# emolch/kiwi

Hardware: AMD Instinct MI355X
Metric: trial-source misfit evals/s (higher is better)
Workload: dtype f32

## Files before the change

### kiwi_amd/csrc/kiwi_accum.hip

```cpp
#include "kiwi_accum_api.hpp"

#if KIWI_ARITH == 0
#define KIWI_ARITH_NS exact
#elif KIWI_ARITH == 1
#define KIWI_ARITH_NS fused
#else
#error "KIWI_ARITH: 0 (exact) or 1 (fused)"
#endif

namespace kiwi {
namespace KIWI_ARITH_NS {

#include "kiwi_accum.inc"

#define KIWI_COMMON_ARGS a.G, a.span, a.pitch, a.recs, a.cent_ofs, a.isrc0, a.nrec, a.recv, a.syn, a.syn_stride

#if KIWI_FAMILY == 1
void launch_direct(const AccumArgs &a, dim3 grid)
{
    if (a.ng == 10) hipLaunchKernelGGL(accumulate_kernel<10>, grid, dim3(256), 0, a.stream, KIWI_COMMON_ARGS, a.synrow);
    else            hipLaunchKernelGGL(accumulate_kernel<8>, grid, dim3(256), 0, a.stream, KIWI_COMMON_ARGS, a.synrow);
}
#endif

// ... 31 lines not shown
template <int NG, int NS, bool COMPACT, bool PLAN>
static void multi_t(const AccumArgs &a, dim3 grid, int ntiles, const int *mate, const int *wider)
{
    if (a.fuse) hipLaunchKernelGGL((accumulate_multi_kernel<NG, true, NS, COMPACT, PLAN>), grid, dim3(256), 0, a.stream, KIWI_COMMON_ARGS, ntiles, a.tab, a.coefs, a.fp,
                                   a.pairflag, mate, wider, a.plan, a.plan_ofs);
    else        hipLaunchKernelGGL((accumulate_multi_kernel<NG, false, NS, COMPACT, PLAN>), grid, dim3(256), 0, a.stream, KIWI_COMMON_ARGS, ntiles, a.tab, a.coefs, a.fp,
                                   a.pairflag, mate, wider, a.plan, a.plan_ofs);
}
template <int NG, int NS>
static void multi_c(const AccumArgs &a, dim3 grid, int ntiles, const int *mate, const int *wider)
{
    if (a.compact && a.plan) multi_t<NG, NS, true, true>(a, grid, ntiles, mate, wider);
    else if (a.compact) multi_t<NG, NS, true, false>(a, grid, ntiles, mate, wider);
    else multi_t<NG, NS, false, false>(a, grid, ntiles, mate, wider);
}
void launch_multi(const AccumArgs &a, dim3 grid, int NS, int ntiles, const int *mate, const int *wider)
{
    if (a.ng == 10) { if (NS == 4) multi_c<10, 4>(a, grid, ntiles, mate, wider); else multi_c<10, 2>(a, grid, ntiles, mate, wider); }
    else            { if (NS == 4) multi_c<8, 4>(a, grid, ntiles, mate, wider); else multi_c<8, 2>(a, grid, ntiles, mate, wider); }
}
void launch_multi_plan(const AccumArgs &a, int NS, int ngroups, const int *mate, const int *wider, PlanSrc *plan)
{
    const dim3 grid((unsigned)ngroups, (unsigned)((a.nrec + 63) / 64));
    if (NS == 4) hipLaunchKernelGGL(multi_plan_kernel<4>, grid, dim3(64), 0, a.stream, a.recs, a.cent_ofs, a.isrc0, a.nrec, a.recv, a.tab, a.pairflag, mate, wider,
                                    a.plan_ofs, (int4 *)plan, a.plan_regular, a.plan_repeat, a.plan_count);
    else         hipLaunchKernelGGL(multi_plan_kernel<2>, grid, dim3(64), 0, a.stream, a.recs, a.cent_ofs, a.isrc0, a.nrec, a.recv, a.tab, a.pairflag, mate, wider,
                                    a.plan_ofs, (int4 *)plan, a.plan_regular, a.plan_repeat, a.plan_count);
}
#endif

#if KIWI_FAMILY == 4
template <int NG, bool COMPACT>
static void cell_t(const AccumArgs &a, dim3 grid, int ntiles, bool per_wave)
{
#define KIWI_C(KERNEL) hipLaunchKernelGGL(KERNEL, grid, dim3(256), 0, a.stream, KIWI_COMMON_ARGS, ntiles, a.tab, a.coefs, a.fp, a.pairflag, a.synrow, \
                                          a.fam_ofs, a.fam_list)
    if (per_wave) { if (a.fuse) KIWI_C((accumulate_cellw_kernel<NG, true, COMPACT>)); else KIWI_C((accumulate_cellw_kernel<NG, false, COMPACT>)); }
    else          { if (a.fuse) KIWI_C((accumulate_cell_kernel<NG, 256, 2, 0, true, COMPACT>)); else KIWI_C((accumulate_cell_kernel<NG, 256, 2, 0, false, COMPACT>)); }
#undef KIWI_C
}
template <int NG>
static void cell_c(const AccumArgs &a, dim3 grid, int ntiles, bool per_wave)
{
    if (a.compact) cell_t<NG, true>(a, grid, ntiles, per_wave); else cell_t<NG, false>(a, grid, ntiles, per_wave);
}
void launch_cell(const AccumArgs &a, dim3 grid, int ntiles) { if (a.ng == 10) cell_c<10>(a, grid, ntiles, false); else cell_c<8>(a, grid, ntiles, false); }
void launch_cellw(const AccumArgs &a, dim3 grid, int ntiles) { if (a.ng == 10) cell_c<10>(a, grid, ntiles, true); else cell_c<8>(a, grid, ntiles, true); }
int cellw_range() { return kCellwRange; }
#endif
// ... 4 lines not shown
```

### kiwi_amd/csrc/kiwi_accum.inc

```


typedef float f4u __attribute__((ext_vector_type(4), aligned(4)));
typedef float f2u __attribute__((ext_vector_type(2), aligned(4)));

#if defined(KIWI_EXPLICIT_FMA)
#ifndef KIWI_CELLW_AHEAD
#define KIWI_CELLW_AHEAD 3
#endif
template <class V> __device__ __forceinline__ V kiwi_mad(V acc, float w, V v)
{
    V ws;
    for (int k = 0; k < (int)(sizeof(V) / sizeof(float)); k++) ws[k] = w;
    return __builtin_elementwise_fma(ws, v, acc);
}
template <class V> __device__ __forceinline__ V kiwi_madv(V acc, V w, V v) { return __builtin_elementwise_fma(w, v, acc); }
#else
template <class V> __device__ __forceinline__ V kiwi_mad(V acc, float w, V v) { return acc + w * v; }
template <class V> __device__ __forceinline__ V kiwi_madv(V acc, V w, V v) { return acc + w * v; }
#endif

typedef int v4i_t __attribute__((ext_vector_type(4)));
typedef int v2i_t __attribute__((ext_vector_type(2)));
__device__ __forceinline__ __amdgpu_buffer_rsrc_t gf_rsrc(const float *base)
{
// ... 256 lines not shown

template <bool BLEND>
__device__ __forceinline__ void pair_finish(const f4u (&v)[2][BLEND ? 4 : 1], float *__restrict__ tile0, int lds_tile, int ig0, int p,
                                            const GeoRec &g)
{
#pragma unroll
    for (int q = 0; q < 2; q++) {
        f4u b;
        if constexpr (BLEND) {
            b = g.w[0] * v[q][0];
            b = b + g.w[1] * v[q][1];
            b = b + g.w[2] * v[q][2];
            b = b + g.w[3] * v[q][3];
        } else {
            b = v[q][0];
        }
        *(float4 *)(tile0 + (ig0 + q) * lds_tile + p) = make_float4(b.x, b.y, b.z, b.w);
    }
}

struct HaloRegs { f4u v[4]; };

struct DescLanes {
    int ta, tb;
    __device__ __forceinline__ int a(int ig, int k) const { return REC_I(ta, 4 * ig + k); }
    __device__ __forceinline__ int b(int ig, int k) const { return REC_I(tb, 4 * ig + k); }
    __device__ __forceinline__ int ha(int hig, int k) const { return __shfl(ta, 4 * hig + k, 64); }
    __device__ __forceinline__ int hb(int hig, int k) const { return __shfl(tb, 4 * hig + k, 64); }
    __device__ __forceinline__ bool fast(int jb, int lds_tile, int pitch, int lane, int ng) const
    {
        const bool lane_ok = lane >= 4 * ng || (ta + jb >= tb && ta + jb + lds_tile <= tb + pitch);
        return __builtin_amdgcn_ballot_w64(lane_ok) == ~0ull;
    }
};
struct DescPlan {
    int b0[4], o[4], pitch, hoff;
    __device__ __forceinline__ int b(int ig, int k) const { return b0[k] + ig * pitch; }
    __device__ __forceinline__ int a(int ig, int k) const { return b0[k] + ig * pitch + o[k]; }
    __device__ __forceinline__ int hb(int, int k) const { return b0[k] + hoff; }
    __device__ __forceinline__ int ha(int, int k) const { return b0[k] + hoff + o[k]; }
    __device__ __forceinline__ bool fast(int jb, int lds_tile, int pitch_, int, int) const
    {
        const int omin = min(min(o[0], o[1]), min(o[2], o[3])), omax = max(max(o[0], o[1]), max(o[2], o[3]));
        return omin + jb >= 0 && omax + jb + lds_tile <= pitch_;
    }
};

template <bool BLEND, bool FAST, typename D>
__device__ __forceinline__ HaloRegs halo_issue(bool active, int ig, int ph, int jb, const float *__restrict__ G, int pitch, const D &d)
{
    HaloRegs h;
#pragma unroll
    for (int k = 0; k < (BLEND ? 4 : 1); k++) {
        const int base = d.ha(ig, k);
        int idx = base + jb + ph;
        if constexpr (!FAST) {
            const int lo = d.hb(ig, k);
            idx = min(max(idx, lo), lo + pitch - 4);
        }
        h.v[k] = f4u{ 0.f, 0.f, 0.f, 0.f };
        if (active) h.v[k] = *(const f4u *)(G + (size_t)(unsigned)idx);
    }
    return h;
}
template <bool BLEND, bool FAST>
__device__ __forceinline__ HaloRegs halo_issue(bool active, int ig, int ph, int jb, const float *__restrict__ G, int pitch,
// ... 836 lines not shown
        const int base = d.a(ig, k);
        if constexpr (FAST) {
            v[k] = buf_load4(gf_rsrc(G), p, base + jb);
        } else {
            const int lo = d.b(ig, k);
            const int idx = min(max(base + j, lo), lo + pitch - 4);
            v[k] = *(const f4u *)(G + (size_t)(unsigned)idx);
        }
    }
}

template <typename D>
__device__ __forceinline__ void one_issue_hidden(f4u (&v)[4], int ig, int p, int jb, const float *__restrict__ G, const D &d)
{
    const size_t gi = (size_t)G;
    const v4i_t rs = { (int)(unsigned)gi, (int)((unsigned)(gi >> 32) & 0xffffu), -1, 0x00020000 };
    const int voff = (int)(4u * (unsigned)p);
#pragma unroll
    for (int k = 0; k < 4; k++) {
        const int soff = (int)(4u * (unsigned)(d.a(ig, k) + jb));
        asm volatile("buffer_load_dwordx4 %0, %1, %2, %3 offen" : "=v"(v[k]) : "v"(voff), "s"(rs), "s"(soff));
    }
}
template <int CNT_FULL, int CNT_SHORT>
__device__ __forceinline__ void vm_wait(f4u (&v)[4], int full )
{
    if constexpr (CNT_FULL == CNT_SHORT)
        asm volatile("s_waitcnt vmcnt(%4)" : "+v"(v[0]), "+v"(v[1]), "+v"(v[2]), "+v"(v[3]) : "n"(CNT_FULL));
    else
        asm volatile("s_cmp_eq_u32 %6, 0\n\ts_cbranch_scc1 1f\n\ts_waitcnt vmcnt(%4)\n\ts_branch 2f\n1:\n\ts_waitcnt vmcnt(%5)\n2:"
                     : "+v"(v[0]), "+v"(v[1]), "+v"(v[2]), "+v"(v[3]) : "n"(CNT_FULL), "n"(CNT_SHORT), "s"(full) : "scc");
}

template <bool BLEND>
__device__ __forceinline__ void one_finish(const f4u (&v)[BLEND ? 4 : 1], float *__restrict__ tile0, int lds_tile, int ig, int p,
                                           const GeoRec &g)
{
    f4u b;
    if constexpr (BLEND) {
        b = g.w[0] * v[0];
        b = b + g.w[1] * v[1];
        b = b + g.w[2] * v[2];
        b = b + g.w[3] * v[3];
    } else {
        b = v[0];
    }
// ... 28 lines not shown
                 "+v"(v.r[2][0]), "+v"(v.r[2][1]), "+v"(v.r[2][2]), "+v"(v.r[2][3]), "+v"(v.r[3][0]), "+v"(v.r[3][1]), "+v"(v.r[3][2]), "+v"(v.r[3][3])
    if constexpr (CNT_FULL == CNT_SHORT)
        asm volatile("s_waitcnt vmcnt(%16)" : KIWI_R16 : "n"(CNT_FULL));
    else
        asm volatile("s_cmp_eq_u32 %18, 0\n\ts_cbranch_scc1 1f\n\ts_waitcnt vmcnt(%16)\n\ts_branch 2f\n1:\n\ts_waitcnt vmcnt(%17)\n2:"
                     : KIWI_R16 : "n"(CNT_FULL), "n"(CNT_SHORT), "s"(full) : "scc");
#undef KIWI_R16
}
__device__ __forceinline__ void mfma_finish(const RowsDw &v, float *__restrict__ dst, const float (&w)[4], bool write)
{
    const f4m negz = { -0.f, -0.f, -0.f, -0.f };
#pragma unroll
    for (int m = 0; m < 4; m++) {
        f4m b = __builtin_amdgcn_mfma_f32_4x4x1f32(v.r[0][m], w[0], negz, 0, 0, 0);
        b = b + __builtin_amdgcn_mfma_f32_4x4x1f32(v.r[1][m], w[1], negz, 0, 0, 0);
        b = b + __builtin_amdgcn_mfma_f32_4x4x1f32(v.r[2][m], w[2], negz, 0, 0, 0);
        b = b + __builtin_amdgcn_mfma_f32_4x4x1f32(v.r[3][m], w[3], negz, 0, 0, 0);
        if (write) *(float4 *)(dst + 64 * m) = make_float4(b.x, b.y, b.z, b.w);
    }
}

template <int NG, int NS> __host__ __device__ constexpr int multi_set_stride() { return NG * (1024 / NS + kHalo) + ((NS == 4 && KIWI_MFMA_BLEND) ? 8 : 0); }

template <int NG, bool FAST, int NS, typename D, typename Shadow>
__device__ __forceinline__ void multi_build(float *__restrict__ tile0, int wv, int lane, int tid, int jb, const float *__restrict__ G,
                                            int pitch, const D &d, const GeoRec (&gw)[NS], int only, bool hact, bool whalo, int hig, int hph,
                                            Shadow shadow)
{
    constexpr int TILE = 1024 / NS, LDS_TILE = TILE + kHalo, DEPTH = 3, SET = multi_set_stride<NG, NS>();
    constexpr int N = (NS == 2) ? NG / 2 : (NG + 3) / 4;
    const int p = (NS == 2) ? 4 * (64 * (wv & 1) + lane) : 4 * lane;
    auto comp = [&](int i) { return (NS == 2) ? 2 * i + (wv >> 1) : wv + 4 * i; };
    HaloRegs hv;
    if (whalo) hv = halo_issue<true, FAST>(true, hig, hph, jb, G, pitch, d);
    const bool last_ok = comp(N - 1) < NG;
    if constexpr (KIWI_MFMA_BLEND && FAST && NS == 4 && KIWI_ARITH == 0) {
        RowsDw v[N];
#pragma unroll
        for (int i = 0; i < DEPTH && i < N; i++) if (i < N - 1 || last_ok) rows_issue_dw(v[i], comp(i), lane, jb, G, d);
        __syncthreads();
        shadow();
        const int me = lane & 3;
        float w[4];
#pragma unroll
        for (int k = 0; k < 4; k++) w[k] = me == 0 ? gw[0].w[k] : (me == 1 ? gw[1].w[k] : (me == 2 ? gw[2].w[k] : gw[3].w[k]));
        float *__restrict__ dst = tile0 + me * SET + 4 * (lane >> 2);
        const bool write = only < 0 || only == me;
#pragma unroll
        for (int i = 0; i < N; i++) {
            __builtin_amdgcn_sched_barrier(0);
            if (i < N - 1 || last_ok) {
                const int behind = (i + DEPTH < N ? i + DEPTH : N) - 1 - i;
                const bool short_ = behind > 0 && i + DEPTH >= N;
                const int lastf = __builtin_amdgcn_readfirstlane(last_ok ? 1 : 0);
                switch (behind) {
                case 0: vm_wait16<0, 0>(v[i], 1); break;
                case 1: if (short_) vm_wait16<16, 0>(v[i], lastf); else vm_wait16<16, 16>(v[i], 1); break;
                default: if (short_) vm_wait16<32, 16>(v[i], lastf); else vm_wait16<32, 32>(v[i], 1); break;
                }
                mfma_finish(v[i], dst + comp(i) * LDS_TILE, w, write);
            }
            if (i + DEPTH < N && (i + DEPTH < N - 1 || last_ok)) rows_issue_dw(v[i + DEPTH], comp(i + DEPTH), lane, jb, G, d);
        }
        if (whalo) {
#pragma unroll
            for (int s = 0; s < NS; s++)
                if (only < 0 || only == s) halo_finish<true>(hact, hv, tile0 + s * SET, LDS_TILE, hig, hph, gw[s]);
        }
        return;
    }
    f4u v[N][4];
    auto issue = [&](int i) __attribute__((always_inline)) {
        if constexpr (FAST) one_issue_hidden(v[i], comp(i), p, jb, G, d);
        else one_issue<true, false>(v[i], comp(i), p, jb, G, pitch, d);
    };
#pragma unroll
    for (int i = 0; i < DEPTH && i < N; i++) if (i < N - 1 || last_ok) issue(i);
    __syncthreads();
    shadow();
#pragma unroll
    for (int i = 0; i < N; i++) {
        __builtin_amdgcn_sched_barrier(0);
        if (i < N - 1 || last_ok) {
            if constexpr (FAST) {
                const int behind = (i + DEPTH < N ? i + DEPTH : N) - 1 - i;
                const bool short_ = behind > 0 && i + DEPTH >= N;
                const int lastf = __builtin_amdgcn_readfirstlane(last_ok ? 1 : 0);
                switch (behind) {
                case 0: vm_wait<0, 0>(v[i], 1); break;
                case 1: if (short_) vm_wait<4, 0>(v[i], lastf); else vm_wait<4, 4>(v[i], 1); break;
                default: if (short_) vm_wait<8, 4>(v[i], lastf); else vm_wait<8, 8>(v[i], 1); break;
                }
            }
#pragma unroll
            for (int s = 0; s < NS; s++)
                if (only < 0 || only == s) one_finish<true>(v[i], tile0 + s * SET, LDS_TILE, comp(i), p, gw[s]);
        }
        if (i + DEPTH < N && (i + DEPTH < N - 1 || last_ok)) issue(i + DEPTH);
    }
    if (whalo) {
#pragma unroll
        for (int s = 0; s < NS; s++)
            if (only < 0 || only == s) halo_finish<true>(hact, hv, tile0 + s * SET, LDS_TILE, hig, hph, gw[s]);
    }
}


__device__ __forceinline__ int smax_u(int a, int b) { int r; asm("s_max_i32 %0, %1, %2" : "=s"(r) : "s"(a), "s"(b) : "scc"); return r; }
__device__ __forceinline__ int smin_u(int a, int b) { int r; asm("s_min_i32 %0, %1, %2" : "=s"(r) : "s"(a), "s"(b) : "scc"); return r; }

template <int NS>
__device__ __forceinline__ bool multi_taken(const RecvDev &rv, const int *__restrict__ pairflag, const int *__restrict__ mate,
                                            int s, int nrec, int r)
{
    if (!mate) return false;
    const int a = s - s % NS;
    if (!mate[a / NS] || !rv.need_h || !rv.has_d) return false;
    int f = 0;
#pragma unroll
    for (int i = 0; i < NS; i++) f |= pairflag[(size_t)(a + i) * nrec + r];
    return f == 0;
}

template <int NS>
__global__ __launch_bounds__(64) void multi_plan_kernel(const GeoRec *__restrict__ recs, const int *__restrict__ cent_ofs, int isrc0, int nrec,
    const RecvDev *__restrict__ recv, const int *__restrict__ off4, const int *__restrict__ pairflag, const int *__restrict__ mate,
    const int *__restrict__ mate_wider, const int *__restrict__ plan_ofs, int4 *__restrict__ plan,
    int regular_on , int repeat_on ,
    unsigned *__restrict__ count )
{
    constexpr int TILE = 1024 / NS, LDS_TILE = TILE + kHalo;
    const int k = (int)blockIdx.x, s0 = NS * k, r = (int)(blockIdx.y * 64 + threadIdx.x);
    if (r >= nrec) return;
    const RecvDev &rv = recv[r];
    if (!rv.enabled) return;
    if (!multi_taken<NS>(rv, pairflag, mate, s0, nrec, r)) return;
    if constexpr (NS == 2) { if (multi_taken<4>(rv, pairflag, mate_wider, s0, nrec, r)) return; }
    const int cb = cent_ofs[isrc0];
    const int nc = cent_ofs[isrc0 + s0 + 1] - cent_ofs[isrc0 + s0];
    const size_t pbeg = (size_t)plan_ofs[k], pend = (size_t)plan_ofs[k + 1];
    size_t pi = pbeg + (size_t)r;
    for (int c = 0; c < nc && pi < pend; pi += (size_t)nrec) {
        const GeoRec *h[NS];
        int smaxs[NS], smins[NS], npos = 0;
        bool shared = true, same_rows = true;
#pragma unroll
        for (int i = 0; i < NS; i++) {
            h[i] = recs + ((size_t)(cent_ofs[isrc0 + s0 + i] - cb) * nrec + (size_t)r * nc + c);
// ... 18 lines not shown
            }
        }
        const int glen = h[0]->pad & 0xff;
        int4 *__restrict__ out = plan + pi * (kPlanStride / 16);
        unsigned nreg = 0, nrep = 0;
#pragma unroll
        for (int i = 0; i < NS; i++) {
            const int4 o = *(const int4 *)(off4 + ((size_t)(cent_ofs[isrc0 + s0 + i] - cb) * nrec + (size_t)r * nc + c) * 4);
            const int e0 = smaxs[i] - h[i]->ishift;
            bool regular = regular_on != 0 && e0 >= 0 && e0 <= kPlanE0Mask;
            bool steps01 = regular && repeat_on != 0 && glen <= 5;
            int repeats = 0;
            for (int j = 1; j < glen && c + j < nc; j++) {
                const int d = h[i][j].ishift - h[i][j - 1].ishift;
                regular = regular && d == 1;
                steps01 = steps01 && (d == 0 || d == 1);
                if (d == 0 && j <= 4) repeats |= 1 << (j - 1);
            }
            if (regular || !steps01) repeats = 0;
            nreg += regular ? 1u : 0u;
            nrep += repeats ? 1u : 0u;
            const int head = (h[i]->flags & 0xffff) | (regular || repeats ? (e0 << kPlanE0Shift) | (regular ? kPlanRegularBit : 0) | (repeats << kPlanRepeatShift) : 0)
                             | (glen << 16) | ((shared ? 1 : 0) << 23) | ((npos - TILE) << 24);
            out[4 * i + 0] = make_int4(h[i]->row[0], h[i]->row[1], h[i]->row[2], h[i]->row[3]);
            out[4 * i + 1] = o;
            out[4 * i + 2] = make_int4(__float_as_int(h[i]->w[0]), __float_as_int(h[i]->w[1]), __float_as_int(h[i]->w[2]), __float_as_int(h[i]->w[3]));
            out[4 * i + 3] = make_int4(smaxs[i], head, __float_as_int(h[i]->cl), __float_as_int(h[i]->sl));
        }
        if (count) { atomicAdd(count, (unsigned)NS); atomicAdd(count + 1, nreg); atomicAdd(count + 2, nrep); }
        if (glen < 1) break;
        c += glen;
    }
}

typedef const __attribute__((address_space(4))) v4i_t *plan_cptr;
template <int NS>
__device__ __forceinline__ int plan_warm(size_t p)
{
    int d;
    if constexpr (NS == 4)
        asm volatile("s_load_dword %0, %1, 0x0\n\ts_load_dword %0, %1, 0x40\n\ts_load_dword %0, %1, 0x80\n\ts_load_dword %0, %1, 0xc0" : "=&s"(d) : "s"(p) : "memory");
    else
        asm volatile("s_load_dword %0, %1, 0x0\n\ts_load_dword %0, %1, 0x40" : "=&s"(d) : "s"(p) : "memory");
    return d;
}

template <int NG, bool FUSE, int NS, bool COMPACT ,
// ... 45 lines not shown
        const long long b = (long long)(cent_ofs[isrc0 + s0 + i] - cb) * nrec + (long long)r * nc;
        rbase[i] = ((long long)__builtin_amdgcn_readfirstlane((int)(b >> 32)) << 32) | (unsigned)__builtin_amdgcn_readfirstlane((int)b);
    }
    auto recs_of = [&](int i) { return recs + (size_t)rbase[i]; };
    auto tab_of = [&](int i) { return tab + (size_t)rbase[i] * (compact ? 4 : 128); };
    int c = 0;
    int cur[NS];
    int ta = 0, tb = 0;
    if constexpr (!PLAN) {
#pragma unroll
        for (int i = 0; i < NS; i++) cur[i] = rec_load(recs_of(i), 0, nc, lane);
        if constexpr (compact) ta = off4_load(tab_of(0), 0, lane);
        else { ta = tab_of(0)[lane]; tb = tab_of(0)[64 + lane]; }
    }
    const int hq = 255 - tid, hch = min(hq / NG, 15), hig = hq % NG, hph = TILE + 4 * hch;
    size_t pcur = 0;
    if constexpr (PLAN) {
        const size_t a = (size_t)plan + ((size_t)plan_ofs[blockIdx.x] + (size_t)r) * kPlanStride;
        pcur = ((size_t)(unsigned)__builtin_amdgcn_readfirstlane((int)(a >> 32)) << 32) | (unsigned)__builtin_amdgcn_readfirstlane((int)a);
    }
    const int pstep = nrec * kPlanStride;
    const int hoff = PLAN ? hig * pitch : 0;
    auto plan4 = [&](int byte) { return *(plan_cptr)(pcur + (size_t)(unsigned)byte); };
    while (c < nc) {
        GeoRec g[NS];
        int smaxs[NS], smins[NS], npos = 0;
        bool shared = true, same_rows = true;
        int glen_p = 0;
        DescPlan dp;
        if constexpr (PLAN) {
            const v4i_t rw = plan4(0), of = plan4(16), tl = plan4(48);
            g[0].row[0] = rw.x;
            dp = DescPlan{ { 0, (rw.y - rw.x) * pitch, (rw.z - rw.x) * pitch, (rw.w - rw.x) * pitch }, { of.x, of.y, of.z, of.w }, pitch, hoff };
            const unsigned head = (unsigned)tl.y;
            glen_p = (int)((head >> 16) & 0x7fu);
            shared = ((head >> 23) & 1u) != 0u;
            npos = TILE + (int)(head >> 24);
            smaxs[0] = tl.x;
        }
        if constexpr (compact && !PLAN) desc_expand(ta, cur[0], lane, pitch, ta, tb);
        if constexpr (!PLAN) {
#pragma unroll
        for (int i = 0; i < NS; i++) {
            g[i].ishift = REC_I(cur[i], 8);
            g[i].pad = REC_I(cur[i], 19);
            smaxs[i] = g[i].ishift + ((g[i].pad >> 8) & 0xff);
            smins[i] = g[i].ishift - ((g[i].pad >> 16) & 0xff);
            npos = max(npos, TILE + (smaxs[i] - smins[i]) + 8);
            if (i == 0) g[0].row[0] = REC_I(cur[0], 0);
            else {
                same_rows = same_rows && (__builtin_amdgcn_ballot_w64(cur[i] != cur[0]) & 0xfull) == 0ull;
                shared = shared && smaxs[i] == smaxs[0];
            }
        }
        shared = shared && same_rows;
        if (same_rows && !shared) {
            int smax_c = smaxs[0], smin_c = smins[0];
#pragma unroll
            for (int i = 1; i < NS; i++) { smax_c = smax_u(smax_c, smaxs[i]); smin_c = smin_u(smin_c, smins[i]); }
            if (TILE + (smax_c - smin_c) + 8 <= LDS_TILE) {
                shared = true;
                npos = TILE + (smax_c - smin_c) + 8;
#pragma unroll
                for (int i = 0; i < NS; i++) smaxs[i] = smax_c;
            }
        }
        }
        const int glen = PLAN ? glen_p : (g[0].pad & 0xff);
        const int cend = c + glen;
        int smax = smaxs[0];
        if constexpr (PLAN) smax = plan4(64 * sh + 48).x;
        else {
#pragma unroll
            for (int i = 1; i < NS; i++) if (sh == i) smax = smaxs[i];
        }
        int flags = 0, ishv = 0, warm_ = 0, pwarm_ = 0;
        float gcl = 0.f, gsl = 0.f;
        const float *__restrict__ coef_grp = nullptr;
        auto shadow = [&]() {
            if constexpr (PLAN) {
#pragma unroll
                for (int i = 0; i < NS; i++) {
                    const v4i_t w = plan4(64 * i + 32);
                    g[i].w[0] = __int_as_float(w.x); g[i].w[1] = __int_as_float(w.y); g[i].w[2] = __int_as_float(w.z); g[i].w[3] = __int_as_float(w.w);
                }
                const v4i_t me = plan4(64 * sh + 48);
                flags = me.y & 0xffff; gcl = __int_as_float(me.z); gsl = __int_as_float(me.w);
                if (c + glen < nc) pwarm_ = plan_warm<NS>(pcur + (size_t)(unsigned)pstep);
            } else {
#pragma unroll
            for (int i = 0; i < NS; i++) { g[i].w[0] = REC_F(cur[i], 4); g[i].w[1] = REC_F(cur[i], 5); g[i].w[2] = REC_F(cur[i], 6); g[i].w[3] = REC_F(cur[i], 7); }
            int curme = cur[0];
#pragma unroll
            for (int i = 1; i < NS; i++) if (sh == i) curme = cur[i];
            flags = REC_I(curme, 18);
            gcl = REC_F(curme, 16); gsl = REC_F(curme, 17);
            }
            if (!(PLAN && (flags & (kPlanRegularBit | kPlanRepeatMask)))) { if (lane < glen) ishv = rc[c + lane].ishift; }
            const size_t crow = (base_me + c) * kCoefLine;
            const unsigned clo = __builtin_amdgcn_readfirstlane((unsigned)crow), chi = __builtin_amdgcn_readfirstlane((unsigned)(crow >> 32));
            coef_grp = coefs + (((size_t)chi << 32) | clo);
            if constexpr (NG == 10) warm_ = coef_warm(coef_grp);
        };
        auto noshadow = []() {};
#define KIWI_MULTI_BUILD(DESC, I0, ONLY, NPOS, SHADOW) do { \
            const int jb_ = t_tile0 - smaxs[I0] - 1;       \
            const float *__restrict__ Gg = G + (size_t)g[I0].row[0] * (size_t)pitch; \
            const bool fast = (DESC).fast(jb_, LDS_TILE, pitch, lane, NG); \
            const bool hact = hq < 16 * NG && hph < (NPOS); \
            const bool whalo = __builtin_amdgcn_ballot_w64(hact) != 0ull; \
            if (fast) multi_build<NG, true, NS>(&tiles[0], wv, lane, tid, jb_, Gg, pitch, DESC, g, ONLY, hact, whalo, hig, hph, SHADOW); \
            else      multi_build<NG, false, NS>(&tiles[0], wv, lane, tid, jb_, Gg, pitch, DESC, g, ONLY, hact, whalo, hig, hph, SHADOW); } while (0)
        __builtin_amdgcn_s_setprio(1);
        if constexpr (PLAN) {
            if (shared) KIWI_MULTI_BUILD(dp, 0, -1, npos, shadow);
            else {
                KIWI_MULTI_BUILD(dp, 0, 0, npos, shadow);
#pragma unroll
                for (int i = 1; i < NS; i++) {
                    const v4i_t rw = plan4(64 * i), of = plan4(64 * i + 16);
                    smaxs[i] = plan4(64 * i + 48).x;
                    g[i].row[0] = rw.x;
                    const DescPlan di{ { 0, (rw.y - rw.x) * pitch, (rw.z - rw.x) * pitch, (rw.w - rw.x) * pitch }, { of.x, of.y, of.z, of.w }, pitch, hoff };
                    KIWI_MULTI_BUILD(di, i, i, npos, noshadow);
                }
            }
            asm volatile("" :: "s"(pwarm_));
            pcur += (size_t)(unsigned)pstep;
        } else {
        if (shared) KIWI_MULTI_BUILD((DescLanes{ ta, tb }), 0, -1, npos, shadow);
        else {
            KIWI_MULTI_BUILD((DescLanes{ ta, tb }), 0, 0, npos, shadow);
#pragma unroll
            for (int i = 1; i < NS; i++) {
                int tai, tbi;
                if constexpr (compact) desc_expand(off4_load(tab_of(i), c, lane), cur[i], lane, pitch, tai, tbi);
                else { tai = tab_of(i)[(size_t)c * 128 + lane]; tbi = tab_of(i)[(size_t)c * 128 + 64 + lane]; }
                g[i].row[0] = REC_I(cur[i], 0);
                KIWI_MULTI_BUILD((DescLanes{ tai, tbi }), i, i, npos, noshadow);
            }
        }
#pragma unroll
        for (int i = 0; i < NS; i++) cur[i] = rec_load(recs_of(i), cend, nc, lane);
        if (cend < nc) {
            if constexpr (compact) ta = off4_load(tab_of(0), cend, lane);
            else { ta = tab_of(0)[(size_t)cend * 128 + lane]; tb = tab_of(0)[(size_t)cend * 128 + 64 + lane]; }
        }
        }
#undef KIWI_MULTI_BUILD
        __syncthreads();
        __builtin_amdgcn_s_setprio(0);
        {
            const unsigned abase = (unsigned)(size_t)(lds_cfp)&tiles[sh * SET + u0];
            if constexpr (NG == 10 || NG == 8) {
                asm volatile("" :: "s"(warm_));
                const float gcl_u = __int_as_float(__builtin_amdgcn_readfirstlane(__float_as_int(gcl))), gsl_u = __int_as_float(__builtin_amdgcn_readfirstlane(__float_as_int(gsl)));
                const size_t cg_ = (size_t)coef_grp;
                const float *__restrict__ coef_u = (const float *)(((size_t)(unsigned)__builtin_amdgcn_readfirstlane((int)(cg_ >> 32)) << 32) | (unsigned)__builtin_amdgcn_readfirstlane((int)cg_));
                const int n = cend - c;
#define KIWI_ASM_ARGS ar1[0], ar1[1], ar2[0], ar2[1], dz[0], dz[1], abase, ishv, smax, n, coef_u, gcl_u, gsl_u
#define KIWI_PLAN_ARGS ar1[0], ar1[1], ar2[0], ar2[1], dz[0], dz[1], abase, ishv, smax, n, coef_u, gcl_u, gsl_u, head_u
                if constexpr (PLAN) {
                    const int head_u = __builtin_amdgcn_readfirstlane(flags);
                    if constexpr (NG == 10) {
                        if (flags & 2) { if constexpr (K == 5) KIWI_APPLY_PLAN(10, 5, rot)(KIWI_PLAN_ARGS); else KIWI_APPLY_PLAN(10, 9, rot)(KIWI_PLAN_ARGS); }
                        else           { if constexpr (K == 5) KIWI_APPLY_PLAN(10, 5, plain)(KIWI_PLAN_ARGS); else KIWI_APPLY_PLAN(10, 9, plain)(KIWI_PLAN_ARGS); }
                    } else {
                        if (flags & 2) { if constexpr (K == 5) KIWI_APPLY_PLAN(8, 5, rot)(KIWI_PLAN_ARGS); else KIWI_APPLY_PLAN(8, 9, rot)(KIWI_PLAN_ARGS); }
                        else           { if constexpr (K == 5) KIWI_APPLY_PLAN(8, 5, plain)(KIWI_PLAN_ARGS); else KIWI_APPLY_PLAN(8, 9, plain)(KIWI_PLAN_ARGS); }
                    }
                } else
                if constexpr (NG == 10) {
                    if (flags & 2) { if constexpr (K == 5) KIWI_APPLY_ASM(10, 5, rot)(KIWI_ASM_ARGS); else KIWI_APPLY_ASM(10, 9, rot)(KIWI_ASM_ARGS); }
                    else           { if constexpr (K == 5) KIWI_APPLY_ASM(10, 5, plain)(KIWI_ASM_ARGS); else KIWI_APPLY_ASM(10, 9, plain)(KIWI_ASM_ARGS); }
                } else {
                    if (flags & 2) { if constexpr (K == 5) KIWI_APPLY_ASM(8, 5, rot)(KIWI_ASM_ARGS); else KIWI_APPLY_ASM(8, 9, rot)(KIWI_ASM_ARGS); }
                    else           { if constexpr (K == 5) KIWI_APPLY_ASM(8, 5, plain)(KIWI_ASM_ARGS); else KIWI_APPLY_ASM(8, 9, plain)(KIWI_ASM_ARGS); }
                }
#undef KIWI_ASM_ARGS
#undef KIWI_PLAN_ARGS
            } else {
            int cc = c, eprev = 0;
            bool have = false;
#define KIWI_C2STEP(LL, HH, RV, CC) do { \
                const int e = smax - __builtin_amdgcn_readlane(ishv, (CC) - c);        \
                const int d = have ? eprev - e : 0x7fff; \
                carry2_apply<NG, RV, K>(ar1, ar2, dz, LL, HH, abase + 4u * (unsigned)e, d, d, coef_grp + (size_t)((CC) - c) * kCoefLine, gcl, gsl); \
                have = true; eprev = e; } while (0)
            if (flags & 2) {
                set2_dead(X); set2_dead(Y);
                for (; cc + 1 < cend; cc += 2) { KIWI_C2STEP(X, Y, true, cc); KIWI_C2STEP(Y, X, true, cc + 1); }
                if (cc < cend) KIWI_C2STEP(X, Y, true, cc);
            } else {
                set2_dead(X); set2_dead(Y);
                for (; cc + 1 < cend; cc += 2) { KIWI_C2STEP(X, Y, false, cc); KIWI_C2STEP(Y, X, false, cc + 1); }
                if (cc < cend) KIWI_C2STEP(X, Y, false, cc);
            }
#undef KIWI_C2STEP
            }
        }
        c = cend;
    }
    {
        const int js = s0 + sh;
        const int tl = tile * TILE + u0;
        if (!FUSE && tl >= rv.wlen) return;
        float *__restrict__ so = syn + (size_t)js * syn_stride + tl;
        float mom = 0.f;
        if constexpr (FUSE) mom = fp.moment[fp.isrc0 + js];
        const bool whole = tile * TILE + TILE <= rv.wlen;
        for (int k = 0; k < rv.ncomp; k++) {
            f2v o01, o23;
            out4(rv.comp[k], rv.sign[k], rv.cl0, rv.sl0, ar1, ar2, dz, o01, o23);
            if constexpr (!FUSE) {
                const float o[4] = { o01.x, o01.y, o23.x, o23.y };
#pragma unroll
                for (int i = 0; i < 4; i++)
                    if (tl + 64 * i < rv.wlen) so[rv.synofs[k] + 64 * i] = o[i];
                continue;
            }
            double acc = fused_acc4(fp, o01, o23, mom, fp.reft + rv.refofs[k] + tl, fp.tw + rv.refofs[k] + tl, tl, rv.wlen, whole);
            acc = wave_reduce_f64(acc, fp.method == 6);
            if (lane == 63)
// ... 575 lines not shown
```

Baseline: 39180.

## Trim scalar work in planned multi-build: precomputed row offsets, linear loads, coef pointer

The plan kernel now stores row deltas already multiplied by the pitch, so the accumulate kernel no longer recomputes them. A linear-descriptor buffer-load path uses scalar offsets precomputed once per group. The per-group coefficient pointer is advanced incrementally instead of being recomputed with readfirstlane, and the last-task flag and halo threshold are hoisted out of the loop. For the plan path, halo weights are reloaded late and the lane activity test is done lazily, and coef warm is disabled by default. Together these aim to cut scalar ALU work and SGPR pressure in the hot loop, at the cost of more template complexity and a changed plan format.

```diff
diff --git a/kiwi_amd/csrc/kiwi_accum.hip b/kiwi_amd/csrc/kiwi_accum.hip
--- a/kiwi_amd/csrc/kiwi_accum.hip
+++ b/kiwi_amd/csrc/kiwi_accum.hip
@@ -77,9 +77,9 @@
 void launch_multi_plan(const AccumArgs &a, int NS, int ngroups, const int *mate, const int *wider, PlanSrc *plan)
 {
     const dim3 grid((unsigned)ngroups, (unsigned)((a.nrec + 63) / 64));
-    if (NS == 4) hipLaunchKernelGGL(multi_plan_kernel<4>, grid, dim3(64), 0, a.stream, a.recs, a.cent_ofs, a.isrc0, a.nrec, a.recv, a.tab, a.pairflag, mate, wider,
+    if (NS == 4) hipLaunchKernelGGL(multi_plan_kernel<4>, grid, dim3(64), 0, a.stream, a.recs, a.cent_ofs, a.isrc0, a.nrec, a.pitch, a.recv, a.tab, a.pairflag, mate, wider,
                                     a.plan_ofs, (int4 *)plan, a.plan_regular, a.plan_repeat, a.plan_count);
-    else         hipLaunchKernelGGL(multi_plan_kernel<2>, grid, dim3(64), 0, a.stream, a.recs, a.cent_ofs, a.isrc0, a.nrec, a.recv, a.tab, a.pairflag, mate, wider,
+    else         hipLaunchKernelGGL(multi_plan_kernel<2>, grid, dim3(64), 0, a.stream, a.recs, a.cent_ofs, a.isrc0, a.nrec, a.pitch, a.recv, a.tab, a.pairflag, mate, wider,
                                     a.plan_ofs, (int4 *)plan, a.plan_regular, a.plan_repeat, a.plan_count);
 }
 #endif
diff --git a/kiwi_amd/csrc/kiwi_accum.inc b/kiwi_amd/csrc/kiwi_accum.inc
--- a/kiwi_amd/csrc/kiwi_accum.inc
+++ b/kiwi_amd/csrc/kiwi_accum.inc
@@ -302,6 +302,7 @@
 struct HaloRegs { f4u v[4]; };
 
 struct DescLanes {
+    static constexpr bool linear = false;
     int ta, tb;
     __device__ __forceinline__ int a(int ig, int k) const { return REC_I(ta, 4 * ig + k); }
     __device__ __forceinline__ int b(int ig, int k) const { return REC_I(tb, 4 * ig + k); }
@@ -313,7 +314,10 @@
         return __builtin_amdgcn_ballot_w64(lane_ok) == ~0ull;
     }
 };
+__device__ __forceinline__ int smax_u(int a, int b) { int r; asm("s_max_i32 %0, %1, %2" : "=s"(r) : "s"(a), "s"(b) : "scc"); return r; }
+__device__ __forceinline__ int smin_u(int a, int b) { int r; asm("s_min_i32 %0, %1, %2" : "=s"(r) : "s"(a), "s"(b) : "scc"); return r; }
 struct DescPlan {
+    static constexpr bool linear = true;
     int b0[4], o[4], pitch, hoff;
     __device__ __forceinline__ int b(int ig, int k) const { return b0[k] + ig * pitch; }
     __device__ __forceinline__ int a(int ig, int k) const { return b0[k] + ig * pitch + o[k]; }
@@ -321,7 +325,7 @@
     __device__ __forceinline__ int ha(int, int k) const { return b0[k] + hoff + o[k]; }
     __device__ __forceinline__ bool fast(int jb, int lds_tile, int pitch_, int, int) const
     {
-        const int omin = min(min(o[0], o[1]), min(o[2], o[3])), omax = max(max(o[0], o[1]), max(o[2], o[3]));
+        const int omin = smin_u(smin_u(o[0], o[1]), smin_u(o[2], o[3])), omax = smax_u(smax_u(o[0], o[1]), smax_u(o[2], o[3]));
         return omin + jb >= 0 && omax + jb + lds_tile <= pitch_;
     }
 };
@@ -1204,6 +1208,17 @@
         asm volatile("buffer_load_dwordx4 %0, %1, %2, %3 offen" : "=v"(v[k]) : "v"(voff), "s"(rs), "s"(soff));
     }
 }
+__device__ __forceinline__ void one_issue_hidden_linear(f4u (&v)[4], int igp , int p, const float *__restrict__ G, const int (&t)[4])
+{
+    const size_t gi = (size_t)G;
+    const v4i_t rs = { (int)(unsigned)gi, (int)((unsigned)(gi >> 32) & 0xffffu), -1, 0x00020000 };
+    const int voff = (int)(4u * (unsigned)p);
+#pragma unroll
+    for (int k = 0; k < 4; k++) {
+        const int soff = (int)(4u * (unsigned)(t[k] + igp));
+        asm volatile("buffer_load_dwordx4 %0, %1, %2, %3 offen" : "=v"(v[k]) : "v"(voff), "s"(rs), "s"(soff));
+    }
+}
 template <int CNT_FULL, int CNT_SHORT>
 __device__ __forceinline__ void vm_wait(f4u (&v)[4], int full )
 {
@@ -1278,18 +1293,42 @@
 
 template <int NG, int NS> __host__ __device__ constexpr int multi_set_stride() { return NG * (1024 / NS + kHalo) + ((NS == 4 && KIWI_MFMA_BLEND) ? 8 : 0); }
 
-template <int NG, bool FAST, int NS, typename D, typename Shadow>
+#ifndef KIWI_MULTI_COEF_WARM
+#define KIWI_MULTI_COEF_WARM 0
+#endif
+
+template <int NG, int NS> __device__ __forceinline__ int multi_last_task(int wv)
+{
+    if constexpr (NS == 2 || NG % 4 == 0) return 1;
+    constexpr int N = (NG + 3) / 4;
+    return (int)((unsigned)(wv + 4 * (N - 1) - NG) >> 31);
+}
+
+template <int NG, bool FAST, int NS, bool RW, typename D, typename Shadow, typename Reweigh>
 __device__ __forceinline__ void multi_build(float *__restrict__ tile0, int wv, int lane, int tid, int jb, const float *__restrict__ G,
                                             int pitch, const D &d, const GeoRec (&gw)[NS], int only, bool hact, bool whalo, int hig, int hph,
-                                            Shadow shadow)
+                                            int lastf , int hq, int npos ,
+                                            Shadow shadow, Reweigh reweigh)
 {
     constexpr int TILE = 1024 / NS, LDS_TILE = TILE + kHalo, DEPTH = 3, SET = multi_set_stride<NG, NS>();
     constexpr int N = (NS == 2) ? NG / 2 : (NG + 3) / 4;
     const int p = (NS == 2) ? 4 * (64 * (wv & 1) + lane) : 4 * lane;
     auto comp = [&](int i) { return (NS == 2) ? 2 * i + (wv >> 1) : wv + 4 * i; };
+    int t[4] = { 0, 0, 0, 0 };
+    if constexpr (FAST && D::linear) {
+#pragma unroll
+        for (int k = 0; k < 4; k++) { t[k] = d.a(0, k) + jb; asm("" : "+s"(t[k])); }
+    }
     HaloRegs hv;
     if (whalo) hv = halo_issue<true, FAST>(true, hig, hph, jb, G, pitch, d);
-    const bool last_ok = comp(N - 1) < NG;
+    auto halo_lanes = [&]() __attribute__((always_inline)) {
+        if constexpr (RW) {
+            int npos_o = npos;
+            asm volatile("" : "+s"(npos_o));
+            return hq < 16 * NG && hph < npos_o;
+        } else return hact;
+    };
+    const bool last_ok = lastf != 0;
     if constexpr (KIWI_MFMA_BLEND && FAST && NS == 4 && KIWI_ARITH == 0) {
         RowsDw v[N];
 #pragma unroll
@@ -1308,7 +1347,6 @@
             if (i < N - 1 || last_ok) {
                 const int behind = (i + DEPTH < N ? i + DEPTH : N) - 1 - i;
                 const bool short_ = behind > 0 && i + DEPTH >= N;
-                const int lastf = __builtin_amdgcn_readfirstlane(last_ok ? 1 : 0);
                 switch (behind) {
                 case 0: vm_wait16<0, 0>(v[i], 1); break;
                 case 1: if (short_) vm_wait16<16, 0>(v[i], lastf); else vm_wait16<16, 16>(v[i], 1); break;
@@ -1319,15 +1357,17 @@
             if (i + DEPTH < N && (i + DEPTH < N - 1 || last_ok)) rows_issue_dw(v[i + DEPTH], comp(i + DEPTH), lane, jb, G, d);
         }
         if (whalo) {
+            const bool hact_l = halo_lanes();
 #pragma unroll
             for (int s = 0; s < NS; s++)
-                if (only < 0 || only == s) halo_finish<true>(hact, hv, tile0 + s * SET, LDS_TILE, hig, hph, gw[s]);
+                if (only < 0 || only == s) halo_finish<true>(hact_l, hv, tile0 + s * SET, LDS_TILE, hig, hph, gw[s]);
         }
         return;
     }
     f4u v[N][4];
     auto issue = [&](int i) __attribute__((always_inline)) {
-        if constexpr (FAST) one_issue_hidden(v[i], comp(i), p, jb, G, d);
+        if constexpr (FAST && D::linear) one_issue_hidden_linear(v[i], comp(i) * pitch, p, G, t);
+        else if constexpr (FAST) one_issue_hidden(v[i], comp(i), p, jb, G, d);
         else one_issue<true, false>(v[i], comp(i), p, jb, G, pitch, d);
     };
 #pragma unroll
@@ -1341,7 +1381,6 @@
             if constexpr (FAST) {
                 const int behind = (i + DEPTH < N ? i + DEPTH : N) - 1 - i;
                 const bool short_ = behind > 0 && i + DEPTH >= N;
-                const int lastf = __builtin_amdgcn_readfirstlane(last_ok ? 1 : 0);
                 switch (behind) {
                 case 0: vm_wait<0, 0>(v[i], 1); break;
                 case 1: if (short_) vm_wait<4, 0>(v[i], lastf); else vm_wait<4, 4>(v[i], 1); break;
@@ -1355,15 +1394,21 @@
         if (i + DEPTH < N && (i + DEPTH < N - 1 || last_ok)) issue(i + DEPTH);
     }
     if (whalo) {
-#pragma unroll
-        for (int s = 0; s < NS; s++)
-            if (only < 0 || only == s) halo_finish<true>(hact, hv, tile0 + s * SET, LDS_TILE, hig, hph, gw[s]);
-    }
-}
-
-
-__device__ __forceinline__ int smax_u(int a, int b) { int r; asm("s_max_i32 %0, %1, %2" : "=s"(r) : "s"(a), "s"(b) : "scc"); return r; }
-__device__ __forceinline__ int smin_u(int a, int b) { int r; asm("s_min_i32 %0, %1, %2" : "=s"(r) : "s"(a), "s"(b) : "scc"); return r; }
+        if constexpr (RW) {
+            GeoRec gl[NS];
+            reweigh(gl);
+            const bool hact_l = halo_lanes();
+#pragma unroll
+            for (int s = 0; s < NS; s++)
+                if (only < 0 || only == s) halo_finish<true>(hact_l, hv, tile0 + s * SET, LDS_TILE, hig, hph, gl[s]);
+        } else {
+#pragma unroll
+            for (int s = 0; s < NS; s++)
+                if (only < 0 || only == s) halo_finish<true>(halo_lanes(), hv, tile0 + s * SET, LDS_TILE, hig, hph, gw[s]);
+        }
+    }
+}
+
 
 template <int NS>
 __device__ __forceinline__ bool multi_taken(const RecvDev &rv, const int *__restrict__ pairflag, const int *__restrict__ mate,
@@ -1379,7 +1424,7 @@
 }
 
 template <int NS>
-__global__ __launch_bounds__(64) void multi_plan_kernel(const GeoRec *__restrict__ recs, const int *__restrict__ cent_ofs, int isrc0, int nrec,
+__global__ __launch_bounds__(64) void multi_plan_kernel(const GeoRec *__restrict__ recs, const int *__restrict__ cent_ofs, int isrc0, int nrec, int pitch,
     const RecvDev *__restrict__ recv, const int *__restrict__ off4, const int *__restrict__ pairflag, const int *__restrict__ mate,
     const int *__restrict__ mate_wider, const int *__restrict__ plan_ofs, int4 *__restrict__ plan,
     int regular_on , int repeat_on ,
@@ -1444,7 +1489,7 @@
             nrep += repeats ? 1u : 0u;
             const int head = (h[i]->flags & 0xffff) | (regular || repeats ? (e0 << kPlanE0Shift) | (regular ? kPlanRegularBit : 0) | (repeats << kPlanRepeatShift) : 0)
                              | (glen << 16) | ((shared ? 1 : 0) << 23) | ((npos - TILE) << 24);
-            out[4 * i + 0] = make_int4(h[i]->row[0], h[i]->row[1], h[i]->row[2], h[i]->row[3]);
+            out[4 * i + 0] = make_int4(h[i]->row[0], (h[i]->row[1] - h[i]->row[0]) * pitch, (h[i]->row[2] - h[i]->row[0]) * pitch, (h[i]->row[3] - h[i]->row[0]) * pitch);
             out[4 * i + 1] = o;
             out[4 * i + 2] = make_int4(__float_as_int(h[i]->w[0]), __float_as_int(h[i]->w[1]), __float_as_int(h[i]->w[2]), __float_as_int(h[i]->w[3]));
             out[4 * i + 3] = make_int4(smaxs[i], head, __float_as_int(h[i]->cl), __float_as_int(h[i]->sl));
@@ -1536,21 +1581,34 @@
     const int pstep = nrec * kPlanStride;
     const int hoff = PLAN ? hig * pitch : 0;
     auto plan4 = [&](int byte) { return *(plan_cptr)(pcur + (size_t)(unsigned)byte); };
+    const float *__restrict__ coef_cur = nullptr;
+    if constexpr (PLAN) {
+        const size_t a = (size_t)(coefs + base_me * kCoefLine);
+        coef_cur = (const float *)(((size_t)(unsigned)__builtin_amdgcn_readfirstlane((int)(a >> 32)) << 32) | (unsigned)__builtin_amdgcn_readfirstlane((int)a));
+    }
+    const int lastf = PLAN ? __builtin_amdgcn_readfirstlane(multi_last_task<NG, NS>(wv)) : 0;
+    const int hq_wave = 64 * (3 - wv);
+    const int hthr = hq_wave < 16 * NG ? 4 * (hq_wave / NG) : 0x7fffffff;
     while (c < nc) {
         GeoRec g[NS];
         int smaxs[NS], smins[NS], npos = 0;
         bool shared = true, same_rows = true;
         int glen_p = 0;
+        int flags = 0, smax = 0;
+        float gcl = 0.f, gsl = 0.f;
         DescPlan dp;
         if constexpr (PLAN) {
-            const v4i_t rw = plan4(0), of = plan4(16), tl = plan4(48);
+            asm volatile("" : "+s"(pcur));
+            const v4i_t rw = plan4(0), of = plan4(16), me = plan4(64 * sh + 48);
             g[0].row[0] = rw.x;
-            dp = DescPlan{ { 0, (rw.y - rw.x) * pitch, (rw.z - rw.x) * pitch, (rw.w - rw.x) * pitch }, { of.x, of.y, of.z, of.w }, pitch, hoff };
-            const unsigned head = (unsigned)tl.y;
+            dp = DescPlan{ { 0, rw.y, rw.z, rw.w }, { of.x, of.y, of.z, of.w }, pitch, hoff };
+            const unsigned head = (unsigned)me.y;
             glen_p = (int)((head >> 16) & 0x7fu);
             shared = ((head >> 23) & 1u) != 0u;
             npos = TILE + (int)(head >> 24);
-            smaxs[0] = tl.x;
+            smax = me.x;
+            flags = me.y & 0xffff; gcl = __int_as_float(me.z); gsl = __int_as_float(me.w);
+            smaxs[0] = plan4(48).x;
         }
         if constexpr (compact && !PLAN) desc_expand(ta, cur[0], lane, pitch, ta, tb);
         if constexpr (!PLAN) {
@@ -1582,15 +1640,13 @@
         }
         const int glen = PLAN ? glen_p : (g[0].pad & 0xff);
         const int cend = c + glen;
-        int smax = smaxs[0];
-        if constexpr (PLAN) smax = plan4(64 * sh + 48).x;
-        else {
+        if constexpr (!PLAN) {
+            smax = smaxs[0];
 #pragma unroll
             for (int i = 1; i < NS; i++) if (sh == i) smax = smaxs[i];
         }
-        int flags = 0, ishv = 0, warm_ = 0, pwarm_ = 0;
-        float gcl = 0.f, gsl = 0.f;
-        const float *__restrict__ coef_grp = nullptr;
+        int ishv = 0, warm_ = 0, pwarm_ = 0;
+        const float *__restrict__ coef_grp = coef_cur;
         auto shadow = [&]() {
             if constexpr (PLAN) {
 #pragma unroll
@@ -1598,8 +1654,6 @@
                     const v4i_t w = plan4(64 * i + 32);
                     g[i].w[0] = __int_as_float(w.x); g[i].w[1] = __int_as_float(w.y); g[i].w[2] = __int_as_float(w.z); g[i].w[3] = __int_as_float(w.w);
                 }
-                const v4i_t me = plan4(64 * sh + 48);
-                flags = me.y & 0xffff; gcl = __int_as_float(me.z); gsl = __int_as_float(me.w);
                 if (c + glen < nc) pwarm_ = plan_warm<NS>(pcur + (size_t)(unsigned)pstep);
             } else {
 #pragma unroll
@@ -1610,21 +1664,35 @@
             flags = REC_I(curme, 18);
             gcl = REC_F(curme, 16); gsl = REC_F(curme, 17);
             }
-            if (!(PLAN && (flags & (kPlanRegularBit | kPlanRepeatMask)))) { if (lane < glen) ishv = rc[c + lane].ishift; }
-            const size_t crow = (base_me + c) * kCoefLine;
-            const unsigned clo = __builtin_amdgcn_readfirstlane((unsigned)crow), chi = __builtin_amdgcn_readfirstlane((unsigned)(crow >> 32));
-            coef_grp = coefs + (((size_t)chi << 32) | clo);
-            if constexpr (NG == 10) warm_ = coef_warm(coef_grp);
+            if (!(PLAN && (flags & (kPlanRegularBit | kPlanRepeatMask)))) { if constexpr (PLAN) asm volatile(""); if (lane < glen) ishv = rc[c + lane].ishift; }
+            if constexpr (!PLAN) {
+                const size_t crow = (base_me + c) * kCoefLine;
+                const unsigned clo = __builtin_amdgcn_readfirstlane((unsigned)crow), chi = __builtin_amdgcn_readfirstlane((unsigned)(crow >> 32));
+                coef_grp = coefs + (((size_t)chi << 32) | clo);
+            }
+            if constexpr (NG == 10 && (!PLAN || KIWI_MULTI_COEF_WARM)) warm_ = coef_warm(coef_grp);
         };
         auto noshadow = []() {};
+        auto reweigh = [&](GeoRec (&gl)[NS]) {
+            if constexpr (PLAN) {
+                size_t q = pcur;
+                asm volatile("" : "+s"(q));
+#pragma unroll
+                for (int i = 0; i < NS; i++) {
+                    const v4i_t w = *(plan_cptr)(q + (size_t)(unsigned)(64 * i + 32));
+                    gl[i].w[0] = __int_as_float(w.x); gl[i].w[1] = __int_as_float(w.y); gl[i].w[2] = __int_as_float(w.z); gl[i].w[3] = __int_as_float(w.w);
+                }
+            }
+        };
 #define KIWI_MULTI_BUILD(DESC, I0, ONLY, NPOS, SHADOW) do { \
             const int jb_ = t_tile0 - smaxs[I0] - 1;       \
             const float *__restrict__ Gg = G + (size_t)g[I0].row[0] * (size_t)pitch; \
             const bool fast = (DESC).fast(jb_, LDS_TILE, pitch, lane, NG); \
-            const bool hact = hq < 16 * NG && hph < (NPOS); \
-            const bool whalo = __builtin_amdgcn_ballot_w64(hact) != 0ull; \
-            if (fast) multi_build<NG, true, NS>(&tiles[0], wv, lane, tid, jb_, Gg, pitch, DESC, g, ONLY, hact, whalo, hig, hph, SHADOW); \
-            else      multi_build<NG, false, NS>(&tiles[0], wv, lane, tid, jb_, Gg, pitch, DESC, g, ONLY, hact, whalo, hig, hph, SHADOW); } while (0)
+            const bool hact = PLAN ? false : hq < 16 * NG && hph < (NPOS); \
+            const bool whalo = PLAN ? (NPOS) - TILE > hthr : __builtin_amdgcn_ballot_w64(hact) != 0ull; \
+            const int lastf_ = PLAN ? lastf : __builtin_amdgcn_readfirstlane(multi_last_task<NG, NS>(wv)); \
+            if (fast) multi_build<NG, true, NS, PLAN>(&tiles[0], wv, lane, tid, jb_, Gg, pitch, DESC, g, ONLY, hact, whalo, hig, hph, lastf_, hq, NPOS, SHADOW, reweigh); \
+            else      multi_build<NG, false, NS, PLAN>(&tiles[0], wv, lane, tid, jb_, Gg, pitch, DESC, g, ONLY, hact, whalo, hig, hph, lastf_, hq, NPOS, SHADOW, reweigh); } while (0)
         __builtin_amdgcn_s_setprio(1);
         if constexpr (PLAN) {
             if (shared) KIWI_MULTI_BUILD(dp, 0, -1, npos, shadow);
@@ -1635,7 +1703,7 @@
                     const v4i_t rw = plan4(64 * i), of = plan4(64 * i + 16);
                     smaxs[i] = plan4(64 * i + 48).x;
                     g[i].row[0] = rw.x;
-                    const DescPlan di{ { 0, (rw.y - rw.x) * pitch, (rw.z - rw.x) * pitch, (rw.w - rw.x) * pitch }, { of.x, of.y, of.z, of.w }, pitch, hoff };
+                    const DescPlan di{ { 0, rw.y, rw.z, rw.w }, { of.x, of.y, of.z, of.w }, pitch, hoff };
                     KIWI_MULTI_BUILD(di, i, i, npos, noshadow);
                 }
             }
@@ -1667,20 +1735,26 @@
         {
             const unsigned abase = (unsigned)(size_t)(lds_cfp)&tiles[sh * SET + u0];
             if constexpr (NG == 10 || NG == 8) {
-                asm volatile("" :: "s"(warm_));
-                const float gcl_u = __int_as_float(__builtin_amdgcn_readfirstlane(__float_as_int(gcl))), gsl_u = __int_as_float(__builtin_amdgcn_readfirstlane(__float_as_int(gsl)));
-                const size_t cg_ = (size_t)coef_grp;
-                const float *__restrict__ coef_u = (const float *)(((size_t)(unsigned)__builtin_amdgcn_readfirstlane((int)(cg_ >> 32)) << 32) | (unsigned)__builtin_amdgcn_readfirstlane((int)cg_));
+                if constexpr (!PLAN || KIWI_MULTI_COEF_WARM) asm volatile("" :: "s"(warm_));
+                float gcl_u = gcl, gsl_u = gsl;
+                if constexpr (!PLAN) { gcl_u = __int_as_float(__builtin_amdgcn_readfirstlane(__float_as_int(gcl))); gsl_u = __int_as_float(__builtin_amdgcn_readfirstlane(__float_as_int(gsl))); }
+                const float *__restrict__ coef_u = coef_grp;
+                if constexpr (!PLAN) {
+                    const size_t cg_ = (size_t)coef_grp;
+                    coef_u = (const float *)(((size_t)(unsigned)__builtin_amdgcn_readfirstlane((int)(cg_ >> 32)) << 32) | (unsigned)__builtin_amdgcn_readfirstlane((int)cg_));
+                }
                 const int n = cend - c;
 #define KIWI_ASM_ARGS ar1[0], ar1[1], ar2[0], ar2[1], dz[0], dz[1], abase, ishv, smax, n, coef_u, gcl_u, gsl_u
 #define KIWI_PLAN_ARGS ar1[0], ar1[1], ar2[0], ar2[1], dz[0], dz[1], abase, ishv, smax, n, coef_u, gcl_u, gsl_u, head_u
                 if constexpr (PLAN) {
-                    const int head_u = __builtin_amdgcn_readfirstlane(flags);
+                    const int head_u = flags;
+                    int rot_v = flags & 2;
+                    asm("" : "+v"(rot_v));
                     if constexpr (NG == 10) {
-                        if (flags & 2) { if constexpr (K == 5) KIWI_APPLY_PLAN(10, 5, rot)(KIWI_PLAN_ARGS); else KIWI_APPLY_PLAN(10, 9, rot)(KIWI_PLAN_ARGS); }
+                        if (rot_v) { if constexpr (K == 5) KIWI_APPLY_PLAN(10, 5, rot)(KIWI_PLAN_ARGS); else KIWI_APPLY_PLAN(10, 9, rot)(KIWI_PLAN_ARGS); }
                         else           { if constexpr (K == 5) KIWI_APPLY_PLAN(10, 5, plain)(KIWI_PLAN_ARGS); else KIWI_APPLY_PLAN(10, 9, plain)(KIWI_PLAN_ARGS); }
                     } else {
-                        if (flags & 2) { if constexpr (K == 5) KIWI_APPLY_PLAN(8, 5, rot)(KIWI_PLAN_ARGS); else KIWI_APPLY_PLAN(8, 9, rot)(KIWI_PLAN_ARGS); }
+                        if (rot_v) { if constexpr (K == 5) KIWI_APPLY_PLAN(8, 5, rot)(KIWI_PLAN_ARGS); else KIWI_APPLY_PLAN(8, 9, rot)(KIWI_PLAN_ARGS); }
                         else           { if constexpr (K == 5) KIWI_APPLY_PLAN(8, 5, plain)(KIWI_PLAN_ARGS); else KIWI_APPLY_PLAN(8, 9, plain)(KIWI_PLAN_ARGS); }
                     }
                 } else
@@ -1713,6 +1787,7 @@
 #undef KIWI_C2STEP
             }
         }
+        if constexpr (PLAN) coef_cur += (size_t)(unsigned)(glen * kCoefLine);
         c = cend;
     }
     {
diff --git a/profiles/multi_build_counts.py b/profiles/multi_build_counts.py
--- /dev/null
+++ b/profiles/multi_build_counts.py
@@ -0,0 +1,121 @@
+#!/usr/bin/env python3
+import json
+import os
+import re
+import subprocess
+import sys
+
+ROOT = os.path.dirname(os.path.dirname(os.path.abspath(__file__)))
+CSRC = os.path.join(ROOT, "kiwi_amd", "csrc")
+KERNELS = ("accumulate_multi_kernel<10, true, 4, true, true>", "accumulate_multi_kernel<10, true, 2, true, true>")
+CLASSES = ("packed", "other_vector", "lane", "scalar_alu", "scalar_load", "vector_load", "lds", "wait", "branch", "barrier")
+
+
+def classify(mn):
+    if mn == "s_barrier":
+        return "barrier"
+    if mn.startswith("v_pk_"):
+        return "packed"
+    if mn.startswith(("v_readlane", "v_readfirstlane", "v_writelane")):
+        return "lane"
+    if mn.startswith("v_"):
+        return "other_vector"
+    if mn.startswith(("s_load_", "s_buffer_load_")):
+        return "scalar_load"
+    if mn.startswith(("s_waitcnt", "s_nop", "s_sleep")):
+        return "wait"
+    if mn.startswith(("s_branch", "s_cbranch", "s_setpc", "s_swappc", "s_call")):
+        return "branch"
+    if mn.startswith("s_"):
+        return "scalar_alu"
+    if mn.startswith(("buffer_", "global_", "flat_", "scratch_")):
+        return "vector_load"
+    if mn.startswith("ds_"):
+        return "lds"
+    return None
+
+
+def mangled_name(kernel, arith):
+    m = re.match(r"accumulate_multi_kernel<(\d+), (true|false), (\d+), (true|false), (true|false)>", kernel)
+    b = lambda s: "Lb1E" if s == "true" else "Lb0E"
+    return "_ZN4kiwi5%s23accumulate_multi_kernelILi%sE%sLi%sE%s%sEEv" % (arith, m.group(1), b(m.group(2)), m.group(3), b(m.group(4)), b(m.group(5)))
+
+
+def instructions(lines):
+    out = []
+    for line in lines:
+        s = line.split(";", 1)[0].strip()
+        if not s or s.startswith((".", "#", "//")) or s.endswith(":"):
+            continue
+        mn = s.split()[0]
+        if classify(mn) is not None:
+            out.append(mn)
+    return out
+
+
+def kernel_counts(text, report, kernel, arith):
+    name = mangled_name(kernel, arith)
+    lines = text.split("\n")
+    beg = next(i for i, l in enumerate(lines) if l.startswith(name) and l.split()[0].endswith(":"))
+    end = next(i for i in range(beg, len(lines)) if lines[i].startswith(".Lfunc_end"))
+    ins = instructions(lines[beg + 1:end])
+    sp = [(i, m) for i, m in enumerate(ins) if m == "s_setprio"]
+    body = lines[beg + 1:end]
+    prio = [l.split(";", 1)[0].split()[1] for l in body if l.split(";", 1)[0].strip().startswith("s_setprio")]
+    assert len(prio) == len(sp)
+    first = next(i for (i, _), p in zip(sp, prio) if p == "1")
+    last = max(i for (i, _), p in zip(sp, prio) if p == "0")
+    assert first < last, "priority raise behind the drop"
+    segs, cur = [], dict.fromkeys(CLASSES, 0)
+    for mn in ins[first + 1:last]:
+        c = classify(mn)
+        if c == "barrier":
+            cur["barrier"] = 1
+            segs.append(cur)
+            cur = dict.fromkeys(CLASSES, 0)
+            continue
+        if mn != "s_setprio":
+            cur[c] += 1
+    segs.append(cur)
+    for s in segs:
+        s["all"] = sum(s[c] for c in CLASSES)
+    total = {c: sum(s[c] for s in segs) for c in CLASSES + ("all",)}
+    whole = dict.fromkeys(CLASSES, 0)
+    for mn in ins:
+        whole[classify(mn)] += 1
+    whole["all"] = len(ins)
+    sym = lines[beg].split()[0].rstrip(":")
+    m = re.search(r"Function Name: %s\b.*\n(?:.*\n){0,16}?.*SGPRs Spill: (\d+)" % re.escape(sym), report)
+    return {"kernel": kernel, "arith": arith, "raise_to_drop": {"segments": segs, "total": total}, "whole_kernel": whole,
+            "priority_raises": prio.count("1"), "priority_drops": prio.count("0"), "spilled_sgprs": int(m.group(1)) if m else -1}
+
+
+def collect():
+    rows = []
+    for ar in ("exact", "fused"):
+        r = subprocess.run(["make", "-s", "-C", CSRC, "asm", "FAMILY=3", "ARITH=%s" % ar, "PYTHON=" + sys.executable], capture_output=True, text=True)
+        if r.returncode != 0:
+            raise RuntimeError("make asm failed:\n" + r.stderr[-2000:])
+        text = open(os.path.join(CSRC, "build", "accum_3_%s.s" % ar)).read()
+        for k in KERNELS:
+            rows.append(kernel_counts(text, r.stderr + r.stdout, k, ar))
+    return rows
+
+
+def main():
+    rows = collect()
+    for r in rows:
+        print("%s  %s  (scalars parked in vector lanes: %d)" % (r["kernel"], r["arith"], r["spilled_sgprs"]))
+        print("  segment      " + " ".join("%12s" % c for c in CLASSES + ("all",)))
+        for i, s in enumerate(r["raise_to_drop"]["segments"]):
+            print("  %-12d " % i + " ".join("%12d" % s[c] for c in CLASSES + ("all",)))
+        print("  raise-drop   " + " ".join("%12d" % r["raise_to_drop"]["total"][c] for c in CLASSES + ("all",)))
+        print("  whole kernel " + " ".join("%12d" % r["whole_kernel"][c] for c in CLASSES + ("all",)))
+    if "--json" in sys.argv:
+        with open(sys.argv[sys.argv.index("--json") + 1], "w") as f:
+            json.dump(rows, f, indent=1)
+            f.write("\n")
+
+
+if __name__ == "__main__":
+    main()
diff --git a/profiles/multi_lean_rate.py b/profiles/multi_lean_rate.py
--- /dev/null
+++ b/profiles/multi_lean_rate.py
@@ -0,0 +1,36 @@
+#!/usr/bin/env python3
+import json
+import os
+
+HERE = os.path.dirname(os.path.abspath(__file__))
+
+
+def main():
+    r = json.load(open(os.path.join(HERE, "multi_lean_rate.json")))
+    print(r["what"])
+    h = r["cfg3_exact"]
+    for side in ("parent", "change"):
+        print("cfg3 exact %-6s ms_per_step %s   avg_launch_ms %s" % (side, " ".join("%.2f" % v for v in h[side + "_ms_per_step"]),
+                                                                    " ".join("%.2f" % v for v in h[side + "_avg_launch_ms"])))
+    print("spread parent %.2f, change %.2f; fastest parent - slowest change %.2f ms: %s (ratio of means %.4f)"
+          % (h["parent_spread_ms"], h["change_spread_ms"], h["fastest_parent_minus_slowest_change_ms"],
+             "a gain" if h["counts_as_gain"] else "NOT a gain", h["ratio_of_means"]))
+    for name, v in r.get("variants_same_session", {}).items():
+        print("variant %-28s ms_per_step %s" % (name, " ".join("%.2f" % x for x in v["ms_per_step"])))
+    for name, v in r.get("other_once_each", {}).items():
+        print("%-14s parent %.2f -> change %.2f ms per step (launch %.2f -> %.2f)" % (name, v["parent"]["ms_per_step"], v["change"]["ms_per_step"],
+                                                                                     v["parent"]["avg_launch_ms"], v["change"]["avg_launch_ms"]))
+    for side, lines in r.get("kernel_trace", {}).items():
+        if isinstance(lines, list):
+            for line in lines:
+                print("kernel trace %-6s %s" % (side, line))
+    c = r.get("counters_per_wave")
+    if c:
+        for k in sorted(c["parent"]):
+            print("%-16s per wave: parent %.1f -> change %.1f" % (k, c["parent"][k], c["change"][k]))
+    for line in r.get("dump_outputs", []):
+        print(line)
+
+
+if __name__ == "__main__":
+    main()
```

After: 39980, median of 6. +2.1%, better.
